# huggingface/parler-tts

Hardware: NVIDIA H100
Metric: audio codec tokens/sec (all codebooks) (higher is better)
Workload: dtype bf16

## Files before the change

### parler_tts_b200/csrc/attention.cu

```cuda
#include <cstdlib>

#include "common.cuh"
#include "kernels.h"
#include "attn_core.cuh"

namespace ptts {

template <typename T>
__global__ void __launch_bounds__(ATT_THREADS) attention_kernel(AttnArgs p) {
  extern __shared__ __align__(16) float sm[];
  pdl_launch_dependents();
  pdl_wait();
  if (p.ctrl != nullptr && p.ctrl->active == 0) return;
  const int per = (p.q_len + (int)gridDim.z - 1) / (int)gridDim.z;
  attention_item<T>(p, blockIdx.y, blockIdx.x, sm, threadIdx.x, [] { __syncthreads(); }, (int)blockIdx.z * per, (int)(blockIdx.z + 1) * per);
}

template <typename T>
__global__ void __launch_bounds__(256) attention_decode_kernel(AttnArgs p) {
  extern __shared__ __align__(128) unsigned char smd[];
  const int warp = threadIdx.x >> 5, lane = threadIdx.x & 31;
  uint64_t* bars = reinterpret_cast<uint64_t*>(smd) + 2 * warp;
  unsigned char* sm_warp = smd + 128 + (size_t)warp * attn_decode_smem_per_warp<T>();
  attention_decode_init_warp(bars, lane);
  pdl_launch_dependents();
  pdl_wait();
  if (p.ctrl != nullptr && p.ctrl->active == 0) return;
  const int pair = warp >> 1, part = warp & 1;
  const int it = blockIdx.x * 4 + pair;
  if (it >= p.B * p.nkv) return;
  int past = p.past_len;
  if (p.past_from_ctrl) past = p.prefix + p.ctrl->cur_len - 1;
  uint32_t parity = 0;
  float* xch = reinterpret_cast<float*>(smd + 128 + (size_t)8 * attn_decode_smem_per_warp<T>()) + pair * 128;
  attention_decode_item_warp<T>(p, it / p.nkv, it % p.nkv, past, sm_warp, bars, lane, parity, part, 2, xch, pair + 1);
}

constexpr int PRE_TC_WARPS = 8;
constexpr int PRE_TC_WARP_BYTES = 2 * ATT_TC_STAGE_BYTES + 768;
__global__ void __launch_bounds__(PRE_TC_WARPS * 32) attention_prefill_tc_kernel(AttnArgs p) {
  extern __shared__ __align__(128) unsigned char smp[];
  const int warp = threadIdx.x >> 5, lane = threadIdx.x & 31;
  uint64_t* bars = reinterpret_cast<uint64_t*>(smp) + 2 * warp;
  unsigned char* ring0 = smp + 128 + (size_t)warp * PRE_TC_WARP_BYTES;
  unsigned char* ring1 = ring0 + ATT_TC_STAGE_BYTES;
  float* fbuf = reinterpret_cast<float*>(ring1 + ATT_TC_STAGE_BYTES);
  attention_decode_init_warp(bars, lane);
  pdl_launch_dependents();
  pdl_wait();
  if (p.ctrl != nullptr && p.ctrl->active == 0) return;
  const int b = blockIdx.y, h = blockIdx.x;
  const int past = p.past_len;
  bf16* kc = reinterpret_cast<bf16*>(p.kcache) + (size_t)b * p.kv_b_stride + (size_t)h * p.kv_h_stride;
  bf16* vc = reinterpret_cast<bf16*>(p.vcache) + (size_t)b * p.kv_b_stride + (size_t)h * p.kv_h_stride;
  if (!p.cross) {
    const bf16* rope_cos = reinterpret_cast<const bf16*>(p.rope_cos);
    const bf16* rope_sin = reinterpret_cast<const bf16*>(p.rope_sin);
    for (int idx = threadIdx.x; idx < p.q_len * 2 * HD; idx += PRE_TC_WARPS * 32) {
      const int j = idx / (2 * HD), e = idx - j * 2 * HD, d = e & (HD - 1);
      const size_t r = (size_t)b * p.q_len + j;
      const int pos = past + j;
      if (e < HD) {
        const bf16* src = reinterpret_cast<const bf16*>(p.knew) + r * p.ldkv + p.k_col0 + h * HD;
        float x = __bfloat162float(src[d]);
        if (p.rope) {
          const float xp = __bfloat162float(src[d < HD / 2 ? d + HD / 2 : d - HD / 2]);
          x = rope_elem<bf16>(x, xp, d, rope_cos + (size_t)pos * HD, rope_sin + (size_t)pos * HD);
        }
// ... 106 lines not shown
```

### parler_tts_b200/csrc/attn_core.cuh

```cuda
#pragma once
#include "common.cuh"
#include "kernels.h"
#include "ptx.cuh"

namespace ptts {

constexpr int ATT_THREADS = 128;
constexpr int ATT_WARPS = 4;
constexpr int HD = PTTS_HEAD_DIM;

template <typename Sync>
__device__ __forceinline__ float block_reduce(float v, float* sh, bool is_max, int tid, Sync sync) {
  const int warp = tid >> 5, lane = tid & 31;
  v = is_max ? warp_max(v) : warp_sum(v);
  sync();
  if (lane == 0) sh[warp] = v;
  sync();
  float r = sh[0];
#pragma unroll
  for (int w = 1; w < ATT_WARPS; w++) r = is_max ? fmaxf(r, sh[w]) : r + sh[w];
  return r;
}

template <typename T>
// ... 125 lines not shown
        }
#pragma unroll
        for (int u = 0; u < 4; u++)
#pragma unroll
          for (int e = 0; e < 8; e++) acc[e] = fmaf(pw[u], vv[u][e], acc[e]);
      }
#pragma unroll
      for (int e = 0; e < 8; e++) {
        acc[e] += __shfl_xor_sync(0xffffffffu, acc[e], 8);
        acc[e] += __shfl_xor_sync(0xffffffffu, acc[e], 16);
      }
      if (lane < 8) {
#pragma unroll
        for (int e = 0; e < 8; e++) red[warp * HD + d0 + e] = acc[e];
      }
      sync();
      if (tid < HD) {
        float o = red[tid] + red[HD + tid] + red[2 * HD + tid] + red[3 * HD + tid];
        o = o / l;
        reinterpret_cast<T*>(p.out)[r * p.ldo + h * HD + tid] = DT<T>::from_f(o);
      }
    }
  }
}

}

namespace ptts {

template <typename T> struct AttChunk { static constexpr int CH = 32; };
template <> struct AttChunk<float> { static constexpr int CH = 16; };

template <typename T, int CH = AttChunk<T>::CH>
__host__ __device__ constexpr int attn_decode_smem_per_warp() {
  return 2 * 2 * CH * HD * (int)sizeof(T) + (3 * HD) * (int)sizeof(float);
}

template <typename T, int CH = AttChunk<T>::CH>
__device__ __forceinline__ void attention_decode_item_warp(const AttnArgs& p, int b, int kvh, int pos, unsigned char* sm_warp, uint64_t* bars,
                                                           int lane, uint32_t& parity, int part = 0, int nparts = 1, float* xch = nullptr,
                                                           int pair_bar = 0) {
  constexpr int STAGE_ELEMS = CH * HD;
  T* kst = reinterpret_cast<T*>(sm_warp);
  T* vst = kst + 2 * STAGE_ELEMS;
  float* qs = reinterpret_cast<float*>(vst + 2 * STAGE_ELEMS);
  float* kn = qs + HD;
  float* vn = kn + HD;
  const T* __restrict__ rope_cos = reinterpret_cast<const T*>(p.rope_cos) + (size_t)pos * HD;
  const T* __restrict__ rope_sin = reinterpret_cast<const T*>(p.rope_sin) + (size_t)pos * HD;
  const int rep = p.nh / p.nkv;
  T* kc = reinterpret_cast<T*>(p.kcache) + (size_t)b * p.kv_b_stride + (size_t)kvh * p.kv_h_stride;
  T* vc = reinterpret_cast<T*>(p.vcache) + (size_t)b * p.kv_b_stride + (size_t)kvh * p.kv_h_stride;
  const int lo = lane, hi = lane + HD / 2;
  const int n_cached = p.cross ? p.kv_len : pos;
  const int n_chunks_all = (n_cached + CH - 1) / CH;
  const int n_chunks = (n_chunks_all > part) ? (n_chunks_all - part + nparts - 1) / nparts : 0;

  auto issue = [&](int i) {
    const int st = i & 1;
    const int t0 = (part + nparts * i) * CH;
    const int n = (n_cached - t0 < CH) ? (n_cached - t0) : CH;
    const uint32_t bar = smem_u32(&bars[st]);
    if (lane == 0) mbar_expect_tx(bar, (uint32_t)(2 * n * HD * sizeof(T)));
    __syncwarp();
    if (lane < 2) {
      const T* src = (lane == 0 ? kc : vc) + (size_t)t0 * HD;
      T* dst = (lane == 0 ? kst : vst) + st * STAGE_ELEMS;
      asm volatile("cp.async.bulk.shared::cluster.global.mbarrier::complete_tx::bytes [%0], [%1], %2, [%3];"
                   ::"r"(smem_u32(dst)), "l"(src), "r"((uint32_t)(n * HD * sizeof(T))), "r"(bar) : "memory");
    }
  };
  auto wait_stage = [&](int st) {
    const uint32_t bar = smem_u32(&bars[st]);
    const uint32_t par = (parity >> st) & 1u;
    uint32_t ok, spins = 0;
    do {
      ok = mbar_try_wait(bar, par);
      if (!ok && ++spins > (1u << 16)) { if (lane == 0) printf("ptts: attention KV mbarrier timeout (cta %d b %d kvh %d stage %d cross %d n_cached %d chunks %d par %u)\n", (int)blockIdx.x, b, kvh, st, p.cross, n_cached, n_chunks, parity); __trap(); }
    } while (!ok);
    parity ^= (1u << st);
  };

  __syncwarp();
  fence_proxy_async_smem();
  if (n_chunks > 0) issue(0);
  if (n_chunks > 1) issue(1);

  const T* q_first = reinterpret_cast<const T*>(p.q) + (size_t)b * p.ldq + p.q_col0 + (size_t)(kvh * rep) * HD;
  const float qf0 = DT<T>::to_f(q_first[lo]), qf1 = DT<T>::to_f(q_first[hi]);
  if (!p.cross && part == 0) {
    const T* ksrc = reinterpret_cast<const T*>(p.knew) + (size_t)b * p.ldkv + p.k_col0 + kvh * HD;
    const T* vsrc = reinterpret_cast<const T*>(p.vnew) + (size_t)b * p.ldkv + p.v_col0 + kvh * HD;
    float x0 = DT<T>::to_f(ksrc[lo]), x1 = DT<T>::to_f(ksrc[hi]);
    if (p.rope) {
      const float y0 = rope_elem<T>(x0, x1, lo, rope_cos, rope_sin);
      const float y1 = rope_elem<T>(x1, x0, hi, rope_cos, rope_sin);
      x0 = y0; x1 = y1;
    }
    const T v0 = vsrc[lo], v1 = vsrc[hi];
    kc[(size_t)pos * p.kv_t_stride + kv_swz(pos, lo)] = DT<T>::from_f(x0);
    kc[(size_t)pos * p.kv_t_stride + kv_swz(pos, hi)] = DT<T>::from_f(x1);
    vc[(size_t)pos * p.kv_t_stride + kv_swz(pos, lo)] = v0;
    vc[(size_t)pos * p.kv_t_stride + kv_swz(pos, hi)] = v1;
    kn[lo] = DT<T>::rnd(x0); kn[hi] = DT<T>::rnd(x1);
    vn[lo] = DT<T>::to_f(v0); vn[hi] = DT<T>::to_f(v1);
  }
  const int grp = lane >> 3, d0 = (lane & 7) * 8;
  const int* km = p.key_mask ? p.key_mask + (size_t)b * p.mask_ld : nullptr;

  for (int rr = 0; rr < rep; rr++) {
    const int h = kvh * rep + rr;
    {
      const T* qsrc = reinterpret_cast<const T*>(p.q) + (size_t)b * p.ldq + p.q_col0 + h * HD;
      float x0 = (rr == 0) ? qf0 : DT<T>::to_f(qsrc[lo]), x1 = (rr == 0) ? qf1 : DT<T>::to_f(qsrc[hi]);
      if (p.rope) {
        const float y0 = rope_elem<T>(x0, x1, lo, rope_cos, rope_sin);
        const float y1 = rope_elem<T>(x1, x0, hi, rope_cos, rope_sin);
        x0 = y0; x1 = y1;
      }
      __syncwarp();
      qs[lo] = x0; qs[hi] = x1;
      __syncwarp();
    }
    float qv[8];
#pragma unroll
    for (int e = 0; e < 8; e++) qv[e] = qs[d0 + e];
    float m_run = -INFINITY, l_run = 0.f;
    float acc[8];
#pragma unroll
    for (int e = 0; e < 8; e++) acc[e] = 0.f;

    auto process = [&](const T* kb, const T* vb, uint32_t mword, int n) {
      constexpr int PER = CH / 4;
      float sloc[PER];
#pragma unroll
      for (int u = 0; u < PER; u++) {
        const int r = u * 4 + grp, rc = r < n ? r : n - 1;
        float kf[8];
        load8(kb + rc * HD + kv_swz(rc, d0), kf);
        float s = 0.f;
#pragma unroll
        for (int e = 0; e < 8; e++) s = fmaf(qv[e], kf[e], s);
        sloc[u] = s;
      }
#pragma unroll
      for (int u = 0; u < PER; u++) sloc[u] += __shfl_xor_sync(0xffffffffu, sloc[u], 1);
#pragma unroll
      for (int u = 0; u < PER; u++) sloc[u] += __shfl_xor_sync(0xffffffffu, sloc[u], 2);
#pragma unroll
      for (int u = 0; u < PER; u++) sloc[u] += __shfl_xor_sync(0xffffffffu, sloc[u], 4);
      float cmax = -INFINITY;
#pragma unroll
      for (int u = 0; u < PER; u++) {
        const int r = u * 4 + grp;
        sloc[u] = (r < n && ((mword >> r) & 1u)) ? sloc[u] * p.scale : -INFINITY;
        cmax = fmaxf(cmax, sloc[u]);
      }
      cmax = warp_max(cmax);
      const float m_new = fmaxf(m_run, cmax);
      if (m_new == -INFINITY) return;
      const float corr = (m_run == -INFINITY) ? 0.f : expf(m_run - m_new);
      l_run *= corr;
#pragma unroll
      for (int e = 0; e < 8; e++) acc[e] *= corr;
      float lsum = 0.f;
#pragma unroll
      for (int u = 0; u < PER; u++) {
        const int r = u * 4 + grp, rc = r < n ? r : n - 1;
        const float pe = expf(sloc[u] - m_new);
        lsum += pe;
        const float pw = DT<T>::rnd(pe);
        float vf[8];
        load8(vb + rc * HD + kv_swz(rc, d0), vf);
#pragma unroll
        for (int e = 0; e < 8; e++) acc[e] = fmaf(pw, vf[e], acc[e]);
      }
      lsum += __shfl_xor_sync(0xffffffffu, lsum, 8);
      lsum += __shfl_xor_sync(0xffffffffu, lsum, 16);
      l_run += lsum;
      m_run = m_new;
    };
    auto mask_bits = [&](int t0) -> int {
      const int t = t0 + lane;
      return (km != nullptr && lane < CH && t < p.mask_len && t < n_cached) ? km[t] : 1;
    };

    if (rr > 0) {
      __syncwarp();
      fence_proxy_async_smem();
      if (n_chunks > 0) issue(0);
      if (n_chunks > 1) issue(1);
    }
    for (int c = 0; c < n_chunks; c++) {
      const int st = c & 1;
      const int t0 = (part + nparts * c) * CH;
      const int n = (n_cached - t0 < CH) ? (n_cached - t0) : CH;
      const int mk = mask_bits(t0);
      wait_stage(st);
      process(kst + st * STAGE_ELEMS, vst + st * STAGE_ELEMS, __ballot_sync(0xffffffffu, mk != 0), n);
      if (c + 2 < n_chunks) {
        __syncwarp();
        fence_proxy_async_smem();
        issue(c + 2);
      }
    }
    if (!p.cross && part == 0) {
      __syncwarp();
      float s = 0.f;
      if (grp == 0) {
#pragma unroll
        for (int e = 0; e < 8; e++) s = fmaf(qv[e], kn[d0 + e], s);
      }
      s += __shfl_xor_sync(0xffffffffu, s, 1);
      s += __shfl_xor_sync(0xffffffffu, s, 2);
      s += __shfl_xor_sync(0xffffffffu, s, 4);
      s = __shfl_sync(0xffffffffu, s, 0) * p.scale;
      if (km != nullptr && pos < p.mask_len && km[pos] == 0) s = -INFINITY;
      const float m_new = fmaxf(m_run, s);
      if (m_new != -INFINITY) {
        const float corr = (m_run == -INFINITY) ? 0.f : expf(m_run - m_new);
        const float pe = (s == -INFINITY) ? 0.f : expf(s - m_new);
        const float pw = DT<T>::rnd(pe);
        l_run = l_run * corr + pe;
#pragma unroll
        for (int e = 0; e < 8; e++) acc[e] = acc[e] * corr + ((grp == 0) ? pw * vn[d0 + e] : 0.f);
        m_run = m_new;
      }
    }
#pragma unroll
    for (int e = 0; e < 8; e++) {
      acc[e] += __shfl_xor_sync(0xffffffffu, acc[e], 8);
      acc[e] += __shfl_xor_sync(0xffffffffu, acc[e], 16);
    }
    if (nparts == 2) {
      if (part == 1) {
        if (lane < 8) {
#pragma unroll
          for (int e = 0; e < 8; e++) xch[d0 + e] = acc[e];
        }
        if (lane == 0) { xch[HD] = m_run; xch[HD + 1] = l_run; }
      }
      asm volatile("bar.sync %0, 64;" ::"r"(pair_bar) : "memory");
      if (part == 0) {
        const float m1 = xch[HD], l1 = xch[HD + 1];
        const float mm = fmaxf(m_run, m1);
        const float c0 = (m_run == -INFINITY) ? 0.f : expf(m_run - mm);
        const float c1 = (m1 == -INFINITY) ? 0.f : expf(m1 - mm);
        l_run = l_run * c0 + l1 * c1;
        if (lane < 8) {
#pragma unroll
          for (int e = 0; e < 8; e++) acc[e] = acc[e] * c0 + xch[d0 + e] * c1;
        }
      }
      asm volatile("bar.sync %0, 64;" ::"r"(pair_bar) : "memory");
    }
    if (lane < 8 && part == 0) {
      float o[8];
      const float inv = (l_run > 0.f) ? 1.0f / l_run : 0.f;
#pragma unroll
      for (int e = 0; e < 8; e++) o[e] = acc[e] * inv;
      store8(reinterpret_cast<T*>(p.out) + (size_t)b * p.ldo + h * HD + d0, o);
    }
  }
}

__device__ __forceinline__ uint32_t att_pack(float lo, float hi) {
  const __nv_bfloat162 v = __floats2bfloat162_rn(lo, hi);
  return *reinterpret_cast<const uint32_t*>(&v);
}

__device__ __forceinline__ float att_ex2(float x) {
  float y;
  asm("ex2.approx.ftz.f32 %0, %1;" : "=f"(y) : "f"(x));
  return y;
}

__device__ __forceinline__ void att_bulk_kv(uint32_t dst, const void* src, uint32_t bytes, uint32_t bar, bool stream) {
  if (stream) bulk_g2s_evict_first(dst, src, bytes, bar);
  else bulk_g2s(dst, src, bytes, bar);
}

constexpr int ATT_TC_CH = 32;
constexpr int ATT_TC_STAGE_BYTES = 2 * ATT_TC_CH * HD * 2;

struct TcItem {
  const bf16* q;
  const bf16* knew;
  const bf16* vnew;
// ... 275 lines not shown
```

### parler_tts_b200/csrc/step.cu

```cuda
#include "attn_core.cuh"
#include "common.cuh"
#include "kernels.h"
#include "ln_stats.cuh"
#include "sample_core.cuh"
#include "ptx.cuh"
#include "step.h"
#include "step_common.cuh"

namespace ptts {

constexpr int ST_THREADS = 256;
constexpr int ST_WARPS = 8;
constexpr int ST_HEADER = 512 + 8 * 32 * 2 * 4 + 256;

__device__ __forceinline__ void mbar_wait(uint64_t* bar, uint32_t parity) {
  uint32_t ok;
  uint32_t spins = 0;
  do {
    ok = mbar_try_wait(bar, parity);
    if (!ok && ++spins > (1u << 22)) { printf("ptts: tile mbarrier timeout (cta %d)\n", (int)blockIdx.x); __trap(); }
  } while (!ok);
}

struct Smem {
// ... 225 lines not shown
          for (int w = 0; w < ST_WARPS; w++) v += red[((size_t)w * 32 + er) * RS + cidx];
          if (d.c1 != nullptr) v = rstd * (v - mean * sm.cvec[cidx]) + sm.cvec[32 + cidx];
          v = DT<bf16>::rnd(v);
          if (d.epi == EPI_ACT) v = apply_act(v, p.act);
          const size_t yo = y_offset(n0 + cidx);
          if (d.epi == EPI_RESIDUAL) v = (j == 0 ? __bfloat162float(__ushort_as_bfloat16(rraw)) : DT<bf16>::to_f(d.R[yo])) + v;
          if (d.epi == EPI_F32) reinterpret_cast<float*>(d.Y)[yo] = v;
          else reinterpret_cast<bf16*>(d.Y)[yo] = __float2bfloat16_rn(v);
        }
      }
    }
    prof_mark(sm.prof, 4);
  }
}

__device__ __forceinline__ void run_gemm(const StepParams& p, Smem& sm, const GemmDesc& d, int nt) {
  switch (nt) {
    case 1: gemm_tasks<1>(p, sm, d); break;
    case 2: gemm_tasks<2>(p, sm, d); break;
    case 3: gemm_tasks<3>(p, sm, d); break;
    default: gemm_tasks<4>(p, sm, d); break;
  }
}

__device__ __forceinline__ void attn_phase(const StepParams& p, Smem& sm, const AttnArgs& a, int nkv, int pos, uint32_t& att_parity, int ph) {
  const int warp = threadIdx.x >> 5, lane = threadIdx.x & 31;
  unsigned char* region = sm.scratch + (size_t)warp * attn_decode_smem_per_warp<bf16>();
  uint64_t* bars = sm.bars + 2 + 2 * warp;
  const int items = p.B * nkv;
  const int pair = warp >> 1, part = warp & 1;
  float* xch = reinterpret_cast<float*>(sm.scratch + (size_t)ST_WARPS * attn_decode_smem_per_warp<bf16>()) + pair * 128;
  __syncthreads();
  for (int it = blockIdx.x + gridDim.x * pair; it < items; it += gridDim.x * (ST_WARPS / 2))
    attention_decode_item_warp<bf16>(a, it / nkv, it % nkv, pos, region, bars, lane, att_parity, part, 2, xch, pair + 1);
}

template <int ITEMS>
__global__ void __launch_bounds__(ST_THREADS, 1) decode_step_kernel(const __grid_constant__ StepParams p) {
  extern __shared__ __align__(128) unsigned char smem_raw[];
  Ctrl* ctrl = p.sa.ctrl;
  if (p.prof != nullptr && blockIdx.x == 0 && threadIdx.x == 0) p.prof[(size_t)(8 * p.L + 2) * 8 + 3] = clock64();
  if (ctrl->active == 0) return;
  const int cur_len = ctrl->cur_len;
  const unsigned gen = (unsigned)ctrl->launch_gen;
  const int pos = p.P + cur_len - 1;
  const int tid = threadIdx.x, warp = tid >> 5, lane = tid & 31;
  const int H = p.H;

  Smem sm;
  sm.bars = reinterpret_cast<uint64_t*>(smem_raw);
  sm.stats = reinterpret_cast<float*>(smem_raw + 256);
  sm.part = reinterpret_cast<float*>(smem_raw + 512);
  sm.cvec = reinterpret_cast<float*>(smem_raw + 2560);
  sm.scratch = smem_raw + ST_HEADER;
  sm.wbuf = reinterpret_cast<const uint4*>(smem_raw + ST_HEADER + p.wbuf_offset);
  sm.pitch = H + 8;
  sm.nbuf = p.nbuf;
  sm.tile0 = reinterpret_cast<bf16*>(sm.scratch);
  sm.parity = 0;
  sm.prof = nullptr;
  if (tid == 0) {
    mbar_init<1>(&sm.bars[0]);
    mbar_init<1>(&sm.bars[1]);
    mbar_init<1>(&sm.bars[WBAR]);
    asm volatile("fence.mbarrier_init.release.cluster;" ::: "memory");
  }
  attention_decode_init_warp(sm.bars + 2 + 2 * warp, lane);
// ... 164 lines not shown
```

### parler_tts_b200/csrc/step2.cu

```cuda
#include "attn_core.cuh"
#include "common.cuh"
#include "kernels.h"
#include "ln_stats.cuh"
#include "sample_core.cuh"
#include "ptx.cuh"
#include "step.h"
#include "step_common.cuh"
#include <type_traits>

namespace ptts {
namespace cl {

constexpr int C = 2;
constexpr int V = 8;
constexpr int THREADS = 256;
constexpr int ROWS = 32;
constexpr int HROWS = 8;
constexpr int ATT_SMEM = attn_decode_smem_per_warp<bf16>();
constexpr int PROF_STRIDE = 16;
constexpr int QMAX = 6;
constexpr int OFF_STATS = 256, OFF_PART = 512, OFF_RES = 2560, OFF_CVEC = 3584;
constexpr int HDR = 5632;
constexpr int WB_BYTES = 65536;
constexpr int R_OFF = HDR + 2 * WB_BYTES;
constexpr int R_BYTES = 92160;
constexpr int R_PASS0 = 65536;
constexpr int QKV_OFF = R_BYTES - 2048;
constexpr int SMEM_BYTES = R_OFF + R_BYTES;
static_assert(SMEM_BYTES + 1024 <= 227 * 1024, "cluster step kernel shared memory");
static_assert(ROWS * (1024 / 2 + 8) * 2 <= V * (256 + ROWS * 34 * 4) && 2 * V * (256 + ROWS * 34 * 4) <= R_BYTES, "fc1 plan");
static_assert(2 * V * C * (32 + 4 * 96 * 4) <= R_PASS0 && R_PASS0 + V * QMAX * 32 * 16 <= QKV_OFF, "QKV plan");
static_assert(5 * ATT_SMEM <= QKV_OFF && 3 * ATT_SMEM <= WB_BYTES && 16384 + 4 * 128 * 4 <= WB_BYTES, "attention plan");
static_assert(ROWS * (4096 / 4 + 8) * 2 + V * (256 + ROWS * 8 * 4) <= R_BYTES, "fc2 plan");

__device__ __forceinline__ void mbar_wait(uint64_t* bar, uint32_t parity, int what) {
  uint32_t ok, spins = 0;
  do {
    ok = mbar_try_wait_cluster(bar, parity);
    if (!ok && ++spins > (1u << 22)) { printf("ptts: cluster step mbarrier timeout (cta %d, barrier kind %d)\n", (int)blockIdx.x, what); __trap(); }
  } while (!ok);
}
__device__ __forceinline__ void bulk_s2peer(uint32_t dst_cluster_addr, const void* src_smem, uint32_t bytes, uint32_t bar_cluster_addr) {
  asm volatile("cp.async.bulk.shared::cluster.shared::cta.mbarrier::complete_tx::bytes [%0], [%1], %2, [%3];"
               ::"r"(dst_cluster_addr), "r"(smem_u32(src_smem)), "r"(bytes), "r"(bar_cluster_addr) : "memory");
}
__device__ __forceinline__ uint32_t mapa(uint32_t addr, uint32_t rank) { uint32_t r; asm volatile("mapa.shared::cluster.u32 %0, %1, %2;" : "=r"(r) : "r"(addr), "r"(rank)); return r; }
__device__ __forceinline__ uint32_t cluster_rank() { uint32_t r; asm volatile("mov.u32 %0, %%cluster_ctarank;" : "=r"(r)); return r; }
__device__ __forceinline__ void cluster_arrive() { asm volatile("barrier.cluster.arrive.release.aligned;" ::: "memory"); }
__device__ __forceinline__ void cluster_wait() { asm volatile("barrier.cluster.wait.acquire.aligned;" ::: "memory"); }
__device__ __forceinline__ void cluster_arrive_reuse() { asm volatile("barrier.cluster.arrive.relaxed.aligned;" ::: "memory"); }

__host__ __device__ __forceinline__ int kslice(int kt) { return (kt & 7) >> 2; }
__host__ __device__ __forceinline__ int klocal(int kt) { return ((kt >> 3) << 2) | (kt & 3); }
__host__ __device__ __forceinline__ int kglobal(int rank, int lk) { return ((lk >> 2) << 3) | (rank << 2) | (lk & 3); }

template <int QN, int MT, bool STATS, bool ACC = false>
__device__ __forceinline__ void mma_slice(float (&out)[2][6][4], RowStatFrag& rst, const bf16* xs, int apitch, const uint4* wb, int KT, int kt0,
                                          int kt_end, int lrow, int lcol) {
  float acc[MT][QN][4];
#pragma unroll
  for (int a = 0; a < MT; a++)
#pragma unroll
    for (int j = 0; j < QN; j++)
#pragma unroll
      for (int e = 0; e < 4; e++) acc[a][j][e] = ACC ? out[a][j][e] : 0.f;
// ... 156 lines not shown
  for (int ph = 0; ph < n_phases; ph++) {
    const int l = ph / 6, sub = ph - 6 * l;
    prof = prof0 ? prof0 + (size_t)(ph + 1) * PROF_STRIDE : nullptr;
    prof_mark(prof, 0);
    const char* lb = blob + p.layer0 + p.layer_stride * l;
    const bool rowpart = (sub == PH_QKV || sub == PH_QC);
    const bool has_ln = (sub == PH_QKV || sub == PH_QC || sub == PH_FC1);
    const int q = (sub == PH_QKV) ? 6 : (sub == PH_QC ? 2 : (sub == PH_FC1 ? qe : 1));
    const int Nc = 4 * q * 8;
    const int KT = (sub == PH_FC2 ? KsF : Ks) >> 5;
    const int apitch = (sub == PH_FC2) ? pitchF : pitch;
    const int act_bytes = (rowpart ? HROWS : ROWS) * apitch * 2;
    const int RS = (q == 1) ? 8 : 8 * q + 2;
    const int blk = rowpart ? 32 + 4 * 16 * q * 4 : 256 + ROWS * RS * 4;
    const int wsend = rowpart ? C * blk : blk;
    const int j0 = JOBS_PER_LAYER * l + (sub == 0 ? 0 : sub + QKV_JOBS - 1);

    float cv1 = 0.f, cv2 = 0.f;
    if (has_ln) {
      const float* c1; int ntot;
      if (sub == PH_QKV) { c1 = reinterpret_cast<const float*>(lb + p.c_qkv); ntot = p.qkv_rows; }
      else if (sub == PH_QC) { c1 = reinterpret_cast<const float*>(lb + p.c_qc); ntot = H; }
      else { c1 = reinterpret_cast<const float*>(lb + p.c_fc1); ntot = F; }
      const int nown = rowpart ? Nc : 8 * q;
      if (tid < nown) {
        int n;
        if (sub == PH_QKV) n = (tid >> 6) * (p.nh * HD) + head * HD + (tid & 63);
        else if (sub == PH_QC) n = head * HD + tid;
        else n = cta * 8 * q + tid;
        cv1 = c1[n];
        cv2 = c1[ntot + n];
      }
    }

    auto wait_job = [&](int j) {
      mbar_wait(&wbar[j & 1], (par_w >> (j & 1)) & 1u, 1);
      par_w ^= 1u << (j & 1);
    };
    auto ring = [&](int j) { return reinterpret_cast<const uint4*>(smem + HDR + (j & 1) * WB_BYTES) + lane; };
    wait_job(j0);
    if (sub == PH_QKV) wait_job(j0 + 1);
    mbar_wait(abar, par_a, 0);
    par_a ^= 1u;
    prof_mark(prof, 1);
    float acc[2][QMAX][4];
    float4* const pass0 = reinterpret_cast<float4*>(Rg + R_PASS0) + (size_t)warp * QMAX * 32 + lane;
    RowStatFrag rst;
    row_stat_zero(rst);
    {
      const bf16* xs = reinterpret_cast<const bf16*>(Rg);
      if (rowpart) {
        auto head_pass = [&](auto pass_tag) {
          constexpr int P = decltype(pass_tag)::value;
          const int u = 2 * P + dgrp;
          float t[2][QMAX][4];
          if (sub == PH_QKV) mma_slice<6, 1, P == 0>(t, rst, xs, apitch, ring(j0 + u), KT, e4, KT, lrow & 7, lcol);
          else mma_slice<2, 1, P == 0>(t, rst, xs, apitch, ring(j0) + (size_t)(2 * u) * KT * 32, KT, e4, KT, lrow & 7, lcol);
#pragma unroll
          for (int j = 0; j < QMAX; j++)
            if (j < q) {
              if (P == 0) pass0[j * 32] = make_float4(t[0][j][0], t[0][j][1], t[0][j][2], t[0][j][3]);
              else {
#pragma unroll
                for (int e = 0; e < 4; e++) acc[0][j][e] = t[0][j][e];
              }
            }
        };
        head_pass(std::integral_constant<int, 0>{});
        if (sub == PH_QKV) {
          __syncthreads();
          if (tid == 0) { issue_weight_job(j0 + 2); issue_weight_job(j0 + 3); }
          wait_job(j0 + 2);
          wait_job(j0 + 3);
        }
        head_pass(std::integral_constant<int, 1>{});
      } else if (sub == PH_FC2) {
        auto quarter = [&](auto qq_tag) {
          constexpr int QQ = decltype(qq_tag)::value;
          const uint4* wq = ring(j0) + (size_t)dgrp * 2 * KT * 32 + (size_t)QQ * KT * 32;
          mma_slice<1, 2, false, QQ == 1>(acc, rst, xs, apitch, wq, 2 * KT, (e4 - QQ * KT) & 3, KT, lrow, lcol);
        };
        quarter(std::integral_constant<int, 0>{});
        __syncthreads();
        if (tid == 0) request_slice(h_img + (size_t)(2 * rank + 1) * h_slice_elems, (uint32_t)(h_slice_elems * 2));
        mbar_wait(abar, par_a, 0);
        par_a ^= 1u;
        quarter(std::integral_constant<int, 1>{});
      } else {
        const uint4* wb = ring(j0) + (size_t)(dgrp * q) * KT * 32;
        if (sub == PH_FC1) {
          if (q == 4) mma_slice<4, 2, true>(acc, rst, xs, apitch, wb, KT, e4, KT, lrow, lcol);
          else if (q == 2) mma_slice<2, 2, true>(acc, rst, xs, apitch, wb, KT, e4, KT, lrow, lcol);
          else mma_slice<1, 2, true>(acc, rst, xs, apitch, wb, KT, e4, KT, lrow, lcol);
        } else mma_slice<1, 2, false>(acc, rst, xs, apitch, wb, KT, e4, KT, lrow, lcol);
      }
    }
    prof_mark(prof, 2);
    if (has_ln && tid < (rowpart ? Nc : 8 * q)) { cvec[tid] = cv1; cvec[256 + tid] = cv2; }
    __syncthreads();
    prof_mark(prof, 12);
    cluster_wait();
    prof_mark(prof, 13);

    const int nslots = rowpart ? V * C : V;
    unsigned char* send = Rg;
    const int send_end = V * wsend;
    unsigned char* recv = Rg + (((send_end > act_bytes ? send_end : act_bytes) + 127) & ~127);
    if (tid == 0) mbar_expect_tx(xbar, (uint32_t)(nslots * blk));
    {
      unsigned char* mine = send + (size_t)warp * wsend;
      if (!rowpart) {
        float* bp = reinterpret_cast<float*>(mine + 256);
#pragma unroll
        for (int mt = 0; mt < 2; mt++)
#pragma unroll
          for (int j = 0; j < QMAX; j++) {
            if (j < q) {
              float* base = bp + (size_t)(mt * 16 + g) * RS + j * 8 + 2 * t4;
              *reinterpret_cast<float2*>(base) = make_float2(acc[mt][j][0], acc[mt][j][1]);
              *reinterpret_cast<float2*>(base + 8 * RS) = make_float2(acc[mt][j][2], acc[mt][j][3]);
            }
          }
        if (has_ln) {
          float* st = reinterpret_cast<float*>(mine);
#pragma unroll
          for (int mt = 0; mt < 2; mt++) {
            const int r0 = mt * 16 + g;
            if (t4 == 0) { st[2 * r0] = rst.s1[mt][0]; st[2 * (r0 + 8)] = rst.s1[mt][2]; }
            if (t4 == (g >> 1)) {
              st[2 * r0 + 1] = (g & 1) ? rst.sq[mt][0][1] : rst.sq[mt][0][0];
              st[2 * (r0 + 8) + 1] = (g & 1) ? rst.sq[mt][1][3] : rst.sq[mt][1][2];
            }
// ... 25 lines not shown
        if (warp < C && lane == 0) {
          fence_proxy_async_smem();
          bulk_s2peer(mapa(smem_u32(recv + (size_t)(8 * rank) * blk), (uint32_t)warp), send + (size_t)warp * V * blk, (uint32_t)(V * blk), mapa(smem_u32(xbar), (uint32_t)warp));
        }
      }
    }
    if (warp == 1 && lane == 0 && !rowpart) issue_weight_job(j0 + 2);
    if (warp == 1 && lane == 0 && sub == PH_QKV) issue_weight_job(j0 + QKV_JOBS);
    prof_mark(prof, 15);
    mbar_wait(xbar, par_x, 2);
    par_x ^= 1u;
    prof_mark(prof, 3);

    if (!rowpart) {
      const int row = tid >> 3, f0 = tid & 7;
      float ln_mean = 0.f, ln_rstd = 0.f;
      if (has_ln) {
        float S1 = 0.f, S2 = 0.f;
#pragma unroll
        for (int v = 0; v < V; v++) { const float2 x = *reinterpret_cast<const float2*>(recv + (size_t)v * blk + row * 8); S1 += x.x; S2 += x.y; }
        ln_mean = S1 / (float)H;
        ln_rstd = rsqrtf(fmaxf(S2 / (float)H - ln_mean * ln_mean, 0.f) + p.eps);
      }
      if (row < B && sub == PH_FC1 && q == 4) {
        const int f = 4 * f0;
        float v[4] = {0.f, 0.f, 0.f, 0.f};
#pragma unroll
        for (int sv = 0; sv < V; sv++) {
          const float* bp = reinterpret_cast<const float*>(recv + (size_t)sv * blk + 256) + row * RS + f;
          const float2 a = *reinterpret_cast<const float2*>(bp), b2 = *reinterpret_cast<const float2*>(bp + 2);
          v[0] += a.x; v[1] += a.y; v[2] += b2.x; v[3] += b2.y;
        }
#pragma unroll
        for (int e = 0; e < 4; e++) v[e] = apply_act(DT<bf16>::rnd(ln_rstd * (v[e] - ln_mean * cvec[f + e]) + cvec[256 + f + e]), p.act);
        uint2 pk;
        pk.x = att_pack(v[0], v[1]); pk.y = att_pack(v[2], v[3]);
        *reinterpret_cast<uint2*>(h_img + h_offset(cta * 32 + f) + row * pitchF) = pk;
      } else if (row < B) {
        for (int i = 0; i < q; i++) {
          const int f = f0 + 8 * i;
          float v = 0.f;
#pragma unroll
          for (int sv = 0; sv < V; sv++) v += reinterpret_cast<const float*>(recv + (size_t)sv * blk + 256)[row * RS + f];
          if (sub == PH_FC1) {
            v = ln_rstd * (v - ln_mean * cvec[f]) + cvec[256 + f];
            v = apply_act(DT<bf16>::rnd(v), p.act);
            h_img[h_offset(cta * 8 * q + f) + row * pitchF] = __float2bfloat16_rn(v);
          } else {
            v = DT<bf16>::rnd(res_s[row * 8 + f] + DT<bf16>::rnd(v));
            res_s[row * 8 + f] = v;
            x_img[(size_t)xo_slice * x_slice_elems + row * pitch + xo_col + f] = __float2bfloat16_rn(v);
          }
        }
      }
    } else {
      bf16* qkv_s = reinterpret_cast<bf16*>(Rg + QKV_OFF);
      auto gather = [&](auto jw_tag) {
        constexpr int JW = decltype(jw_tag)::value, NC = 4 * JW, QCW = 2 * JW;
        for (int idx = tid; idx < 4 * NC; idx += THREADS) {
          const int r4 = idx / NC, col = idx - r4 * NC;
          const int u = col / JW, cw = (u >> 1) * JW + (col - u * JW);
          float S1 = 0.f, S2 = 0.f;
#pragma unroll
          for (int e = 0; e < V; e++) {
            const float2 x = *reinterpret_cast<const float2*>(recv + (size_t)(8 * (e >> 2) + 2 * (e & 3)) * blk + r4 * 8);
            S1 += x.x; S2 += x.y;
          }
          const float ln_mean = S1 / (float)H;
          const float ln_rstd = rsqrtf(fmaxf(S2 / (float)H - ln_mean * ln_mean, 0.f) + p.eps);
          float v = 0.f;
#pragma unroll
          for (int e = 0; e < V; e++)
            v += reinterpret_cast<const float*>(recv + (size_t)(8 * (e >> 2) + 2 * (e & 3) + (u & 1)) * blk + 32)[r4 * QCW + cw];
          v = ln_rstd * (v - ln_mean * cvec[col]) + cvec[256 + col];
          qkv_s[idx] = __float2bfloat16_rn(v);
        }
      };
      if (sub == PH_QKV) gather(std::integral_constant<int, 48>{}); else gather(std::integral_constant<int, 16>{});
      static_assert(HD == 64, "QKV: 2 x 2 units of 6 n-tiles (q|k|v of a head), q_cross: 2 x 2 units of 2 n-tiles");
    }
    prof_mark(prof, 4);
    __syncthreads();
    cluster_arrive_reuse();
    if (rowpart) {
      cluster_wait();
      cluster_arrive();
    }

    if (rowpart) {
      if (att_row < B) {
        AttnArgs att = decode_attn_args(p, l, pos, sub == PH_QC);
        const bf16* qkv_s = reinterpret_cast<const bf16*>(Rg + QKV_OFF);
        const int row_base = HROWS * rblk + 4 * rank;
        const bf16* qbase = qkv_s - (size_t)row_base * Nc - (size_t)head * HD;
        att.q = qbase; att.ldq = Nc;
        att.ldo = pitch;
        att.out = a_img + (size_t)att_slice * x_slice_elems + att_col - (size_t)head * HD;
        if (sub == PH_QKV) { att.knew = qbase; att.vnew = qbase; att.ldkv = Nc; att.k_col0 = HD; att.v_col0 = 2 * HD; }
        unsigned char* wb0 = smem + HDR;
        unsigned char* held = wb0 + ((sub == PH_QKV ? j0 + 1 : j0) & 1) * WB_BYTES;
        unsigned char* other = wb0 + ((sub == PH_QKV ? j0 : j0 + 1) & 1) * WB_BYTES;
        unsigned char* region = warp < 5 ? Rg + (size_t)warp * ATT_SMEM : held + (size_t)(warp - 5) * ATT_SMEM;
        float* xr = reinterpret_cast<float*>(other + 16384) + (warp >> 1) * 128;
        attention_decode_item_warp<bf16>(att, att_row, head, pos, region, attbars + 2 * warp, lane, att_parity, warp & 1, 2, xr, (warp >> 1) + 1);
      }
      prof_mark(prof, 5);
      __syncthreads();
      if (tid == 32) {
        fence_proxy_async_smem();
        issue_weight_job(sub == PH_QKV ? j0 + QKV_JOBS + 1 : j0 + 2);
      }
    }
    prof_mark(prof, 6);
    if (p.prof != nullptr && l == p.L / 2 && tid == 0) {
      unsigned long long ns;
      asm volatile("mov.u64 %0, %%globaltimer;" : "=l"(ns));
      p.prof[(size_t)(n_phases + 4) * PROF_STRIDE + sub * (int)gridDim.x + cta] = (long long)ns;
    }

    const bool last = (ph + 1 == n_phases);
    const bf16* nimg; uint32_t nbytes;
    if (last) { nimg = x_img; nbytes = (uint32_t)(C * x_slice_elems * 2); }
    else slice_of((sub + 1) % 6, nimg, nbytes);
    bar_target = grid_sync(bar_ctr, bar_target, ph, false, nullptr, [&]() { request_slice(nimg, nbytes); });
    prof_mark(prof, 7);
  }
  cluster_wait();

  prof = prof0 ? prof0 + (size_t)(n_phases + 1) * PROF_STRIDE : nullptr;
  prof_mark(prof, 0);
  {
    const int ntasks = p.K * p.V / 32;
    const float* c1 = reinterpret_cast<const float*>(blob + p.c_heads);
    const float* c2 = c1 + p.K * p.V;
    mbar_wait(abar, par_a, 3);
    par_a ^= 1u;
    const bf16* xs = reinterpret_cast<const bf16*>(Rg);
// ... 41 lines not shown
#pragma unroll
          for (int j = 0; j < 2; j++) ldmatrix_x4(a[mt][j], sl + (size_t)(mt * 16 + lrow) * pitch + j * 16 + lcol);
#pragma unroll
        for (int j = 0; j < 4; j++) {
          const uint4 w = wb[((size_t)j * KTH + kt) * 32];
#pragma unroll
          for (int mt = 0; mt < 2; mt++) {
            mma_bf16_16816(acc[mt][j], a[mt][0], w.x, w.y);
            mma_bf16_16816(acc[mt][j], a[mt][1], w.z, w.w);
          }
        }
      }
      __syncthreads();
      float* red = reinterpret_cast<float*>(wbuf);
#pragma unroll
      for (int mt = 0; mt < 2; mt++)
#pragma unroll
        for (int j = 0; j < 4; j++) {
          float* base = red + ((size_t)warp * 32 + mt * 16 + g) * HRS + j * 8 + 2 * t4;
          *reinterpret_cast<float2*>(base) = make_float2(acc[mt][j][0], acc[mt][j][1]);
          *reinterpret_cast<float2*>(base + 8 * HRS) = make_float2(acc[mt][j][2], acc[mt][j][3]);
        }
      __syncthreads();
      {
        const int er = tid >> 3, ec = tid & 7;
        if (er < B) {
          const float mean = stats[2 * er], rstd = stats[2 * er + 1];
#pragma unroll
          for (int j = 0; j < 4; j++) {
            const int cidx = j * 8 + ec, n = task * 32 + cidx;
            float v = 0.f;
#pragma unroll
            for (int w = 0; w < 8; w++) v += red[((size_t)w * 32 + er) * HRS + cidx];
            p.logits[(size_t)er * p.K * p.V + n] = DT<bf16>::rnd(rstd * (v - mean * c1[n]) + c2[n]);
          }
        }
      }
      __syncthreads();
      if (tid == 32) {
        fence_proxy_async_smem();
        issue_weight_job(job + 2);
      }
    }
  }
  prof_mark(prof, 6);
  bar_target = grid_sync(bar_ctr, bar_target, n_phases, true);
  prof = prof0 ? prof0 + (size_t)(n_phases + 2) * PROF_STRIDE : nullptr;
  prof_mark(prof, 0);
  if (p.do_sample_phase) {
    const ptts_gen_params gp = *p.sa.gen;
    const int BK = B * p.K;
    sample_phase<ITEMS>(p.sa, gp, BK, cur_len);
    prof_mark(prof, 1);
    bar_target = grid_sync(bar_ctr, bar_target, n_phases + 1, true, nullptr, [&]() {
      const int tot = *reinterpret_cast<volatile int*>(&ctrl->n_unfinished);
      s_next_active = (tot - unfinished_prev > 0) ? 1 : 0;
      unfinished_prev = tot;
    });
    prof_mark(prof, 2);
  }
  bool go_on = false;
  if (p.do_sample_phase) {
    const int act = s_next_active;
    if (cta == 0 && tid == 0) {
      ctrl->cur_len = cur_len + 1;
      ctrl->active = act;
      ctrl->steps_run += 1;
// ... 95 lines not shown
```

Before: 219,700.

## Pre-issue first KV chunk bulk copy before attention in fused decode step

Splits the per-warp attention scratch into separate ring0/ring1/fbuf pointers so the first K/V chunk's bulk async copy can be issued early. For the q_cross phase it is issued right at phase start, and for QKV it is issued after the LN stats sync, so it overlaps the projection GEMM and cluster wait. The shared-memory layout is re-planned so the stage buffers do not collide with the weight buffers. It also rewrites several online-softmax and layernorm expressions as explicit fused multiply-adds and adds optional clock64 profiling hooks that compile out by default. The risk is aliasing between the early-issued copy and buffers that are still live.

```diff
diff --git a/parler_tts_b200/csrc/attention.cu b/parler_tts_b200/csrc/attention.cu
--- a/parler_tts_b200/csrc/attention.cu
+++ b/parler_tts_b200/csrc/attention.cu
@@ -33,7 +33,8 @@
   if (p.past_from_ctrl) past = p.prefix + p.ctrl->cur_len - 1;
   uint32_t parity = 0;
   float* xch = reinterpret_cast<float*>(smd + 128 + (size_t)8 * attn_decode_smem_per_warp<T>()) + pair * 128;
-  attention_decode_item_warp<T>(p, it / p.nkv, it % p.nkv, past, sm_warp, bars, lane, parity, part, 2, xch, pair + 1);
+  attention_decode_item_warp<T>(p, it / p.nkv, it % p.nkv, past, sm_warp, sm_warp + attn_decode_stage_bytes<T>(),
+                                reinterpret_cast<float*>(sm_warp + 2 * attn_decode_stage_bytes<T>()), bars, lane, parity, part, 2, xch, pair + 1);
 }
 
 constexpr int PRE_TC_WARPS = 8;
diff --git a/parler_tts_b200/csrc/attn_core.cuh b/parler_tts_b200/csrc/attn_core.cuh
--- a/parler_tts_b200/csrc/attn_core.cuh
+++ b/parler_tts_b200/csrc/attn_core.cuh
@@ -181,20 +181,49 @@
 template <> struct AttChunk<float> { static constexpr int CH = 16; };
 
 template <typename T, int CH = AttChunk<T>::CH>
+__host__ __device__ constexpr int attn_decode_stage_bytes() {
+  return 2 * CH * HD * (int)sizeof(T);
+}
+template <typename T, int CH = AttChunk<T>::CH>
 __host__ __device__ constexpr int attn_decode_smem_per_warp() {
-  return 2 * 2 * CH * HD * (int)sizeof(T) + (3 * HD) * (int)sizeof(float);
+  return 2 * attn_decode_stage_bytes<T, CH>() + (3 * HD) * (int)sizeof(float);
+}
+
+template <typename T, int CH>
+__device__ __forceinline__ void attention_decode_issue_chunk(const T* kc, const T* vc, int t0, int n, unsigned char* stage, uint64_t* bar, int lane) {
+  const uint32_t b = smem_u32(bar);
+  if (lane == 0) mbar_expect_tx(b, (uint32_t)(2 * n * HD * sizeof(T)));
+  __syncwarp();
+  if (lane < 2) {
+    const T* src = (lane == 0 ? kc : vc) + (size_t)t0 * HD;
+    T* dst = reinterpret_cast<T*>(stage) + (lane == 0 ? 0 : CH * HD);
+    asm volatile("cp.async.bulk.shared::cluster.global.mbarrier::complete_tx::bytes [%0], [%1], %2, [%3];"
+                 ::"r"(smem_u32(dst)), "l"(src), "r"((uint32_t)(n * HD * sizeof(T))), "r"(b) : "memory");
+  }
 }
 
 template <typename T, int CH = AttChunk<T>::CH>
-__device__ __forceinline__ void attention_decode_item_warp(const AttnArgs& p, int b, int kvh, int pos, unsigned char* sm_warp, uint64_t* bars,
-                                                           int lane, uint32_t& parity, int part = 0, int nparts = 1, float* xch = nullptr,
-                                                           int pair_bar = 0) {
+__device__ __forceinline__ void attention_decode_issue_first(const AttnArgs& p, int b, int kvh, int pos, unsigned char* ring0, uint64_t* bars,
+                                                             int lane, int part) {
+  const int n_cached = p.cross ? p.kv_len : pos;
+  const int t0 = part * CH;
+  if (t0 >= n_cached) return;
+  const T* kc = reinterpret_cast<const T*>(p.kcache) + (size_t)b * p.kv_b_stride + (size_t)kvh * p.kv_h_stride;
+  const T* vc = reinterpret_cast<const T*>(p.vcache) + (size_t)b * p.kv_b_stride + (size_t)kvh * p.kv_h_stride;
+  __syncwarp();
+  attention_decode_issue_chunk<T, CH>(kc, vc, t0, (n_cached - t0 < CH) ? (n_cached - t0) : CH, ring0, &bars[0], lane);
+}
+
+template <typename T, int CH = AttChunk<T>::CH>
+__device__ __forceinline__ void attention_decode_item_warp(const AttnArgs& p, int b, int kvh, int pos, unsigned char* ring0, unsigned char* ring1,
+                                                           float* fbuf, uint64_t* bars, int lane, uint32_t& parity, int part = 0, int nparts = 1,
+                                                           float* xch = nullptr, int pair_bar = 0, long long* prof = nullptr,
+                                                           bool pre_issued = false) {
   constexpr int STAGE_ELEMS = CH * HD;
-  T* kst = reinterpret_cast<T*>(sm_warp);
-  T* vst = kst + 2 * STAGE_ELEMS;
-  float* qs = reinterpret_cast<float*>(vst + 2 * STAGE_ELEMS);
+  float* qs = fbuf;
   float* kn = qs + HD;
   float* vn = kn + HD;
+  auto kstage = [&](int st) { return reinterpret_cast<const T*>(st ? ring1 : ring0); };
   const T* __restrict__ rope_cos = reinterpret_cast<const T*>(p.rope_cos) + (size_t)pos * HD;
   const T* __restrict__ rope_sin = reinterpret_cast<const T*>(p.rope_sin) + (size_t)pos * HD;
   const int rep = p.nh / p.nkv;
@@ -208,16 +237,7 @@
   auto issue = [&](int i) {
     const int st = i & 1;
     const int t0 = (part + nparts * i) * CH;
-    const int n = (n_cached - t0 < CH) ? (n_cached - t0) : CH;
-    const uint32_t bar = smem_u32(&bars[st]);
-    if (lane == 0) mbar_expect_tx(bar, (uint32_t)(2 * n * HD * sizeof(T)));
-    __syncwarp();
-    if (lane < 2) {
-      const T* src = (lane == 0 ? kc : vc) + (size_t)t0 * HD;
-      T* dst = (lane == 0 ? kst : vst) + st * STAGE_ELEMS;
-      asm volatile("cp.async.bulk.shared::cluster.global.mbarrier::complete_tx::bytes [%0], [%1], %2, [%3];"
-                   ::"r"(smem_u32(dst)), "l"(src), "r"((uint32_t)(n * HD * sizeof(T))), "r"(bar) : "memory");
-    }
+    attention_decode_issue_chunk<T, CH>(kc, vc, t0, (n_cached - t0 < CH) ? (n_cached - t0) : CH, st ? ring1 : ring0, &bars[st], lane);
   };
   auto wait_stage = [&](int st) {
     const uint32_t bar = smem_u32(&bars[st]);
@@ -232,7 +252,7 @@
 
   __syncwarp();
   fence_proxy_async_smem();
-  if (n_chunks > 0) issue(0);
+  if (!pre_issued && n_chunks > 0) issue(0);
   if (n_chunks > 1) issue(1);
 
   const T* q_first = reinterpret_cast<const T*>(p.q) + (size_t)b * p.ldq + p.q_col0 + (size_t)(kvh * rep) * HD;
@@ -256,6 +276,7 @@
   }
   const int grp = lane >> 3, d0 = (lane & 7) * 8;
   const int* km = p.key_mask ? p.key_mask + (size_t)b * p.mask_ld : nullptr;
+  if (prof != nullptr && lane == 0) prof[8] = clock64();
 
   for (int rr = 0; rr < rep; rr++) {
     const int h = kvh * rep + rr;
@@ -309,7 +330,6 @@
       const float m_new = fmaxf(m_run, cmax);
       if (m_new == -INFINITY) return;
       const float corr = (m_run == -INFINITY) ? 0.f : expf(m_run - m_new);
-      l_run *= corr;
 #pragma unroll
       for (int e = 0; e < 8; e++) acc[e] *= corr;
       float lsum = 0.f;
@@ -326,7 +346,7 @@
       }
       lsum += __shfl_xor_sync(0xffffffffu, lsum, 8);
       lsum += __shfl_xor_sync(0xffffffffu, lsum, 16);
-      l_run += lsum;
+      l_run = __fmaf_rn(l_run, corr, lsum);
       m_run = m_new;
     };
     auto mask_bits = [&](int t0) -> int {
@@ -346,13 +366,15 @@
       const int n = (n_cached - t0 < CH) ? (n_cached - t0) : CH;
       const int mk = mask_bits(t0);
       wait_stage(st);
-      process(kst + st * STAGE_ELEMS, vst + st * STAGE_ELEMS, __ballot_sync(0xffffffffu, mk != 0), n);
+      if (prof != nullptr && lane == 0 && c == 0) prof[19] = clock64();
+      process(kstage(st), kstage(st) + STAGE_ELEMS, __ballot_sync(0xffffffffu, mk != 0), n);
       if (c + 2 < n_chunks) {
         __syncwarp();
         fence_proxy_async_smem();
         issue(c + 2);
       }
     }
+    if (prof != nullptr && lane == 0) { prof[9] = clock64(); prof[11] = n_chunks; }
     if (!p.cross && part == 0) {
       __syncwarp();
       float s = 0.f;
@@ -370,9 +392,9 @@
         const float corr = (m_run == -INFINITY) ? 0.f : expf(m_run - m_new);
         const float pe = (s == -INFINITY) ? 0.f : expf(s - m_new);
         const float pw = DT<T>::rnd(pe);
-        l_run = l_run * corr + pe;
-#pragma unroll
-        for (int e = 0; e < 8; e++) acc[e] = acc[e] * corr + ((grp == 0) ? pw * vn[d0 + e] : 0.f);
+        l_run = __fmaf_rn(l_run, corr, pe);
+#pragma unroll
+        for (int e = 0; e < 8; e++) acc[e] = __fmaf_rn(acc[e], corr, (grp == 0) ? __fmul_rn(pw, vn[d0 + e]) : 0.f);
         m_run = m_new;
       }
     }
@@ -395,14 +417,15 @@
         const float mm = fmaxf(m_run, m1);
         const float c0 = (m_run == -INFINITY) ? 0.f : expf(m_run - mm);
         const float c1 = (m1 == -INFINITY) ? 0.f : expf(m1 - mm);
-        l_run = l_run * c0 + l1 * c1;
+        l_run = __fmaf_rn(l_run, c0, __fmul_rn(l1, c1));
         if (lane < 8) {
 #pragma unroll
-          for (int e = 0; e < 8; e++) acc[e] = acc[e] * c0 + xch[d0 + e] * c1;
+          for (int e = 0; e < 8; e++) acc[e] = __fmaf_rn(acc[e], c0, __fmul_rn(xch[d0 + e], c1));
         }
       }
       asm volatile("bar.sync %0, 64;" ::"r"(pair_bar) : "memory");
     }
+    if (prof != nullptr && lane == 0) prof[10] = clock64();
     if (lane < 8 && part == 0) {
       float o[8];
       const float inv = (l_run > 0.f) ? 1.0f / l_run : 0.f;
diff --git a/parler_tts_b200/csrc/step.cu b/parler_tts_b200/csrc/step.cu
--- a/parler_tts_b200/csrc/step.cu
+++ b/parler_tts_b200/csrc/step.cu
@@ -281,7 +281,9 @@
   float* xch = reinterpret_cast<float*>(sm.scratch + (size_t)ST_WARPS * attn_decode_smem_per_warp<bf16>()) + pair * 128;
   __syncthreads();
   for (int it = blockIdx.x + gridDim.x * pair; it < items; it += gridDim.x * (ST_WARPS / 2))
-    attention_decode_item_warp<bf16>(a, it / nkv, it % nkv, pos, region, bars, lane, att_parity, part, 2, xch, pair + 1);
+    attention_decode_item_warp<bf16>(a, it / nkv, it % nkv, pos, region, region + attn_decode_stage_bytes<bf16>(),
+                                     reinterpret_cast<float*>(region + 2 * attn_decode_stage_bytes<bf16>()), bars, lane, att_parity, part, 2,
+                                     xch, pair + 1);
 }
 
 template <int ITEMS>
diff --git a/parler_tts_b200/csrc/step2.cu b/parler_tts_b200/csrc/step2.cu
--- a/parler_tts_b200/csrc/step2.cu
+++ b/parler_tts_b200/csrc/step2.cu
@@ -16,8 +16,15 @@
 constexpr int THREADS = 256;
 constexpr int ROWS = 32;
 constexpr int HROWS = 8;
-constexpr int ATT_SMEM = attn_decode_smem_per_warp<bf16>();
+#ifdef PTTS_PROFILE_PHASES
+constexpr int PROF_STRIDE = 24;
+#define PROF_PHASE_MARK(slot) prof_mark(prof, slot)
+#define PROF_ATTN (warp == 0 ? prof : nullptr)
+#else
 constexpr int PROF_STRIDE = 16;
+#define PROF_PHASE_MARK(slot) ((void)0)
+#define PROF_ATTN nullptr
+#endif
 constexpr int QMAX = 6;
 constexpr int OFF_STATS = 256, OFF_PART = 512, OFF_RES = 2560, OFF_CVEC = 3584;
 constexpr int HDR = 5632;
@@ -30,7 +37,12 @@
 static_assert(SMEM_BYTES + 1024 <= 227 * 1024, "cluster step kernel shared memory");
 static_assert(ROWS * (1024 / 2 + 8) * 2 <= V * (256 + ROWS * 34 * 4) && 2 * V * (256 + ROWS * 34 * 4) <= R_BYTES, "fc1 plan");
 static_assert(2 * V * C * (32 + 4 * 96 * 4) <= R_PASS0 && R_PASS0 + V * QMAX * 32 * 16 <= QKV_OFF, "QKV plan");
-static_assert(5 * ATT_SMEM <= QKV_OFF && 3 * ATT_SMEM <= WB_BYTES && 16384 + 4 * 128 * 4 <= WB_BYTES, "attention plan");
+constexpr int ATT_STAGE = attn_decode_stage_bytes<bf16>();
+constexpr int QC_STAGE0 = 17408;
+constexpr int ATT_XCH = 49152;
+static_assert(V * ATT_STAGE <= R_PASS0 && V * ATT_STAGE <= WB_BYTES && R_PASS0 + V * 3 * HD * 4 <= QKV_OFF, "attention plan");
+static_assert(2 * V * C * (32 + 4 * 32 * 4) <= QC_STAGE0 && QC_STAGE0 + 5 * ATT_STAGE <= R_PASS0 && QC_STAGE0 % 128 == 0, "q_cross plan");
+static_assert(16384 + 3 * ATT_STAGE <= ATT_XCH && ATT_XCH + 4 * 128 * 4 <= WB_BYTES, "q_cross plan: out-proj jobs of at most 16 KB");
 static_assert(ROWS * (4096 / 4 + 8) * 2 + V * (256 + ROWS * 8 * 4) <= R_BYTES, "fc2 plan");
 
 __device__ __forceinline__ void mbar_wait(uint64_t* bar, uint32_t parity, int what) {
@@ -253,6 +265,14 @@
         cv2 = c1[ntot + n];
       }
     }
+
+    auto held = [&]() { return smem + HDR + ((sub == PH_QKV ? j0 + 1 : j0) & 1) * WB_BYTES; };
+    auto other = [&]() { return smem + HDR + ((sub == PH_QKV ? j0 : j0 + 1) & 1) * WB_BYTES; };
+    auto att_ring0 = [&]() {
+      return sub == PH_QKV ? held() + warp * ATT_STAGE : (warp < 5 ? Rg + QC_STAGE0 + warp * ATT_STAGE : other() + 16384 + (warp - 5) * ATT_STAGE);
+    };
+    if (sub == PH_QC && att_row < B)
+      attention_decode_issue_first<bf16>(decode_attn_args(p, l, pos, true), att_row, head, pos, att_ring0(), attbars + 2 * warp, lane, warp & 1);
 
     auto wait_job = [&](int j) {
       mbar_wait(&wbar[j & 1], (par_w >> (j & 1)) & 1u, 1);
@@ -288,12 +308,14 @@
             }
         };
         head_pass(std::integral_constant<int, 0>{});
+        PROF_PHASE_MARK(16);
         if (sub == PH_QKV) {
           __syncthreads();
           if (tid == 0) { issue_weight_job(j0 + 2); issue_weight_job(j0 + 3); }
           wait_job(j0 + 2);
           wait_job(j0 + 3);
         }
+        PROF_PHASE_MARK(17);
         head_pass(std::integral_constant<int, 1>{});
       } else if (sub == PH_FC2) {
         auto quarter = [&](auto qq_tag) {
@@ -319,6 +341,8 @@
     prof_mark(prof, 2);
     if (has_ln && tid < (rowpart ? Nc : 8 * q)) { cvec[tid] = cv1; cvec[256 + tid] = cv2; }
     __syncthreads();
+    if (sub == PH_QKV && att_row < B)
+      attention_decode_issue_first<bf16>(decode_attn_args(p, l, pos, false), att_row, head, pos, att_ring0(), attbars + 2 * warp, lane, warp & 1);
     prof_mark(prof, 12);
     cluster_wait();
     prof_mark(prof, 13);
@@ -410,7 +434,7 @@
           v[0] += a.x; v[1] += a.y; v[2] += b2.x; v[3] += b2.y;
         }
 #pragma unroll
-        for (int e = 0; e < 4; e++) v[e] = apply_act(DT<bf16>::rnd(ln_rstd * (v[e] - ln_mean * cvec[f + e]) + cvec[256 + f + e]), p.act);
+        for (int e = 0; e < 4; e++) v[e] = apply_act(DT<bf16>::rnd(__fmaf_rn(ln_rstd, __fmaf_rn(-ln_mean, cvec[f + e], v[e]), cvec[256 + f + e])), p.act);
         uint2 pk;
         pk.x = att_pack(v[0], v[1]); pk.y = att_pack(v[2], v[3]);
         *reinterpret_cast<uint2*>(h_img + h_offset(cta * 32 + f) + row * pitchF) = pk;
@@ -421,7 +445,7 @@
 #pragma unroll
           for (int sv = 0; sv < V; sv++) v += reinterpret_cast<const float*>(recv + (size_t)sv * blk + 256)[row * RS + f];
           if (sub == PH_FC1) {
-            v = ln_rstd * (v - ln_mean * cvec[f]) + cvec[256 + f];
+            v = __fmaf_rn(ln_rstd, __fmaf_rn(-ln_mean, cvec[f], v), cvec[256 + f]);
             v = apply_act(DT<bf16>::rnd(v), p.act);
             h_img[h_offset(cta * 8 * q + f) + row * pitchF] = __float2bfloat16_rn(v);
           } else {
@@ -450,7 +474,7 @@
 #pragma unroll
           for (int e = 0; e < V; e++)
             v += reinterpret_cast<const float*>(recv + (size_t)(8 * (e >> 2) + 2 * (e & 3) + (u & 1)) * blk + 32)[r4 * QCW + cw];
-          v = ln_rstd * (v - ln_mean * cvec[col]) + cvec[256 + col];
+          v = __fmaf_rn(ln_rstd, __fmaf_rn(-ln_mean, cvec[col], v), cvec[256 + col]);
           qkv_s[idx] = __float2bfloat16_rn(v);
         }
       };
@@ -463,6 +487,7 @@
     if (rowpart) {
       cluster_wait();
       cluster_arrive();
+      PROF_PHASE_MARK(18);
     }
 
     if (rowpart) {
@@ -475,12 +500,11 @@
         att.ldo = pitch;
         att.out = a_img + (size_t)att_slice * x_slice_elems + att_col - (size_t)head * HD;
         if (sub == PH_QKV) { att.knew = qbase; att.vnew = qbase; att.ldkv = Nc; att.k_col0 = HD; att.v_col0 = 2 * HD; }
-        unsigned char* wb0 = smem + HDR;
-        unsigned char* held = wb0 + ((sub == PH_QKV ? j0 + 1 : j0) & 1) * WB_BYTES;
-        unsigned char* other = wb0 + ((sub == PH_QKV ? j0 : j0 + 1) & 1) * WB_BYTES;
-        unsigned char* region = warp < 5 ? Rg + (size_t)warp * ATT_SMEM : held + (size_t)(warp - 5) * ATT_SMEM;
-        float* xr = reinterpret_cast<float*>(other + 16384) + (warp >> 1) * 128;
-        attention_decode_item_warp<bf16>(att, att_row, head, pos, region, attbars + 2 * warp, lane, att_parity, warp & 1, 2, xr, (warp >> 1) + 1);
+        unsigned char* ring1 = sub == PH_QKV ? Rg + warp * ATT_STAGE : held() + warp * ATT_STAGE;
+        float* fbuf = reinterpret_cast<float*>(Rg + R_PASS0) + warp * 3 * HD;
+        float* xr = reinterpret_cast<float*>(other() + ATT_XCH) + (warp >> 1) * 128;
+        attention_decode_item_warp<bf16>(att, att_row, head, pos, att_ring0(), ring1, fbuf, attbars + 2 * warp, lane, att_parity, warp & 1, 2, xr,
+                                         (warp >> 1) + 1, PROF_ATTN, true);
       }
       prof_mark(prof, 5);
       __syncthreads();
@@ -588,7 +612,7 @@
             float v = 0.f;
 #pragma unroll
             for (int w = 0; w < 8; w++) v += red[((size_t)w * 32 + er) * HRS + cidx];
-            p.logits[(size_t)er * p.K * p.V + n] = DT<bf16>::rnd(rstd * (v - mean * c1[n]) + c2[n]);
+            p.logits[(size_t)er * p.K * p.V + n] = DT<bf16>::rnd(__fmaf_rn(rstd, __fmaf_rn(-mean, c1[n], v), c2[n]));
           }
         }
       }
```

After: 227,800, median of 6. +3.7%, better.
